# Dhole/collaborative_filtering

Hardware: AMD Instinct MI355X
Metric: user-subgraph eigendecomps/sec + predicted ratings/sec, 1M users avg deg 100 (higher is better)
Workload: dtype f32 (eigen) / f64 (predict)

## Files before the change

### collaborative_filtering_amd/_native.py

```python
from __future__ import annotations

import ctypes
import os
from ctypes import POINTER, c_char_p, c_double, c_float, c_int, c_int32, c_uint32, c_uint64, c_void_p

_HERE = os.path.dirname(os.path.abspath(__file__))
LIB_PATH = os.environ.get("CF_MI355X_LIB") or os.path.join(_HERE, "libcf_mi355x.so")
HOST_LIB_PATH = os.path.join(_HERE, "libcf_host.so")

CF_OK = 0
CF_EINVAL = -1
CF_ERANGE = -4
CF_SVD_MAX_NV = 256
CF_ALS_MAX_D = 64
CF_TOPN_MAX_N = 1024
CF_SIGS_OWN = 0
CF_SIGS_COMPAT = 1
CF_MAX_K = 192
CF_SPILL_MAX_K = 5000
CF_EIGEN_TRIDIAG = 0
CF_EIGEN_JACOBI = 1
CF_GRAPH_DENSE = 0
CF_GRAPH_CSR = 1
CF_FILTER_CHEBY = 0
CF_FILTER_BINOMIAL = 1

SIGNATURES = {
    "cf_version": (c_int, []),
    "cf_device_count": (c_int, []),
    "cf_create": (c_int, [c_int, POINTER(c_void_p)]),
    "cf_destroy": (None, [c_void_p]),
    "cf_release_workspaces": (c_int, [c_void_p]),
    "cf_last_error": (c_char_p, [c_void_p]),
    "cf_set_jacobi": (c_int, [c_void_p, c_float, c_int]),
    "cf_set_eigen_refine": (c_int, [c_void_p, c_int, c_float, c_float]),
    "cf_set_eigen_split": (c_int, [c_void_p, c_int]),
    "cf_set_pred_pack": (c_int, [c_void_p, c_int]),
    "cf_debug_split_schedule": (c_int, [c_int, c_int, POINTER(c_int), POINTER(c_int), POINTER(c_int), POINTER(c_int)]),
    "cf_set_step_masks": (c_int, [c_void_p, c_int]),
    "cf_set_local_wlim": (c_int, [c_void_p, c_int]),
    "cf_debug_predict_nmax": (c_int, [c_int]),
    "cf_set_knn2_topk": (c_int, [c_void_p, c_uint32]),
    "cf_set_eigen_method": (c_int, [c_void_p, c_int]),
    "cf_debug_stats": (c_int, [c_void_p, c_int, c_void_p]),
    "cf_eigen_bucket_timing": (c_int, [c_void_p, c_int, c_void_p]),
    "cf_eigen_bucket_timing_split": (c_int, [c_void_p, c_int, c_void_p, c_void_p]),
    "cf_debug_phases": (c_int, [c_void_p, c_int, c_void_p]),
    "cf_debug_spill": (c_int, [c_void_p, c_int, c_void_p]),
    "cf_debug_tri": (c_int, [c_void_p, c_int, c_void_p]),
    "cf_item_graph_upload": (c_int, [c_void_p, c_uint32, c_void_p, c_void_p, c_void_p]),
    "cf_item_graph_upload_dense": (c_int, [c_void_p, c_uint32, c_void_p, c_int]),
    "cf_item_graph_device": (c_void_p, [c_void_p, POINTER(c_uint32)]),
    "cf_set_graph_layout": (c_int, [c_void_p, c_int]),
    "cf_graph_info": (c_int, [c_void_p, c_void_p, c_void_p, c_void_p]),
    "cf_item_cosine_edges": (c_int, [c_void_p, c_uint32, c_uint32, c_void_p, c_void_p, c_void_p, c_float, c_int, c_int,
                                     c_void_p, c_void_p, c_void_p, c_uint64, c_void_p]),
    "cf_plan_create": (c_int, [c_void_p, c_uint32, c_void_p, POINTER(c_void_p)]),
    "cf_plan_destroy": (None, [c_void_p]),
    "cf_evec_slots": (c_uint64, [c_uint32]),
# ... 189 lines not shown
```

### collaborative_filtering_amd/api.py

```python
from __future__ import annotations

from ctypes import byref, c_double, c_float, c_int, c_uint32, c_void_p
from dataclasses import dataclass

import numpy as np

from . import _native
from ._native import CF_ERANGE, CF_FILTER_BINOMIAL, CF_FILTER_CHEBY, CF_SIGS_COMPAT, CF_SIGS_OWN, NativeError, ptr


def _check(lib, ctx, rc, what):
    if rc != _native.CF_OK:
        msg = lib.cf_last_error(ctx)
        raise NativeError(f"{what} failed ({rc}): {msg.decode() if msg else ''}")


def evec_offsets(item_off: np.ndarray) -> tuple[np.ndarray, int]:
    k = np.diff(item_off.astype(np.int64))
    slots = k * np.maximum(k, 2)
    off = np.zeros(len(k), dtype=np.uint64)
    if len(k):
        off[1:] = np.cumsum(slots)[:-1]
    return off, int(slots.sum())

# ... 211 lines not shown
        self.close()

    def __del__(self):
        try:
            self.close()
        except Exception:
            pass

    def _chk(self, rc, what):
        _check(self.lib, self.h, rc, what)

    def set_eigen_method(self, method: str = "jacobi"):
        code = {"tridiag": _native.CF_EIGEN_TRIDIAG, "jacobi": _native.CF_EIGEN_JACOBI}[method]
        self._chk(self.lib.cf_set_eigen_method(self.h, code), "cf_set_eigen_method")

    def set_jacobi(self, tol_scale: float = 1.0, max_sweeps: int = 30):
        self._chk(self.lib.cf_set_jacobi(self.h, tol_scale, max_sweeps), "cf_set_jacobi")

    def set_eigen_refine(self, enable: bool = True, stop_rel: float = 1e-3, delta: float = 1e-2):
        self._chk(self.lib.cf_set_eigen_refine(self.h, int(enable), stop_rel, delta), "cf_set_eigen_refine")

    def set_eigen_split(self, enable=True):
        self._chk(self.lib.cf_set_eigen_split(self.h, int(enable)), "cf_set_eigen_split")

    def set_pred_pack(self, mode=1):
        self._chk(self.lib.cf_set_pred_pack(self.h, int(mode)), "cf_set_pred_pack")

    def set_local_wlim(self, bisect: bool = True):
        self._chk(self.lib.cf_set_local_wlim(self.h, int(bisect)), "cf_set_local_wlim")

    def set_step_masks(self, enable: bool = True):
        self._chk(self.lib.cf_set_step_masks(self.h, int(enable)), "cf_set_step_masks")

    def debug_stats(self, enable: bool = True, read: bool = False):
        out = np.zeros(8, dtype=np.uint64) if read else None
        self._chk(self.lib.cf_debug_stats(self.h, int(enable), ptr(out)), "cf_debug_stats")
        if read:
            n = max(int(out[1]), 1)
            return {"sweeps_mean": int(out[0]) / n, "users": int(out[1]), "sweeps_max": int(out[2]),
                    "capped": int(out[3]), "assembly_cyc_per_user": int(out[4]) / n,
                    "jacobi_cyc_per_user": int(out[5]) / n, "epilogue_cyc_per_user": int(out[6]) / n,
                    "jacobi_cyc_per_step": int(out[5]) / max(int(out[7]), 1)}
        return None

    def eigen_bucket_timing(self, enable: bool = True, read: bool = False, sweeps: bool = False):
        out = np.zeros(13, dtype=np.float32) if read else None
# ... 795 lines not shown
```

### collaborative_filtering_amd/csrc/cf_eigen.hip

```cpp

#include "cf_eigen_common.h"

namespace {
using namespace cf_eig;

template <int EMAX, bool NARROW = false>
struct EigenGeom {
    static constexpr int NR = 16 * EMAX;
    static constexpr int NC = NARROW ? 188 : NR;
    static constexpr int E2 = NR / (2 * kGroup);
    static constexpr int LD16 = NR + ((16 - NR) % 64 + 64) % 64;
    static constexpr int LD = (NC * LD16 + 9 * NR <= 40960 - 4) ? LD16 : NR + 8;
    static constexpr int NT = (NR > 128) ? 1024 : 512;
    static constexpr int WPE = EMAX <= 5 ? 6 : 4;

    static constexpr size_t bytes() {
        return sizeof(float) * (size_t)NC * LD
               + sizeof(uint32_t) * NR
               + sizeof(float) * NR * 5
               + sizeof(int) * NR
               + sizeof(int) * 4;
    }
};
static_assert(EigenGeom<12, true>::LD % 64 == 16, "narrow bucket-12 layout must be conflict-free");
static_assert(EigenGeom<12, true>::bytes() <= 163840, "narrow bucket-12 layout exceeds 160 KiB LDS");

template <int EMAX, bool NARROW = false, bool RESUME = false>
__global__ __launch_bounds__((EigenGeom<EMAX, NARROW>::NT), (EigenGeom<EMAX, NARROW>::WPE)) void eigen_kernel(EigenArgs a) {
    using G = EigenGeom<EMAX, NARROW>;
    constexpr int NR = G::NR;
    constexpr int LD = G::LD;
    auto bidx = [](int i, int j) { return j * LD + i; };
    constexpr int E2 = G::E2;
    constexpr int NT = G::NT;
    extern __shared__ float smem[];
    float* B = smem;
    uint32_t* s_item = reinterpret_cast<uint32_t*>(B + (size_t)G::NC * LD);
    float* s_s = reinterpret_cast<float*>(s_item + NR);
    float* s_l2d = s_s + NR;
    float* s_sig = s_l2d + NR;
    float* s_mu = s_sig + NR;
    float* s_dev = s_mu + NR;
    int* s_perm = reinterpret_cast<int*>(s_dev + NR);
    int* s_flag = s_perm + NR;

    const int tid = threadIdx.x;
    const int lane = tid & 63;
    const int wave = tid >> 6;
    constexpr int NW = NT / 64;
    unsigned long long t_phase0 = (a.stats && tid == 0) ? __builtin_amdgcn_s_memtime() : 0ull;
    unsigned long long t_phase1 = 0, t_phase2 = 0;
    const int mode = a.mode;
    if (a.only_flag && !a.only_flag[blockIdx.x]) return;
    const uint32_t unit = a.order[a.first + blockIdx.x];
// ... 99 lines not shown
            const float si = s_s[i];
            for (int j = lane; j < k; j += 64)
                L2m[(size_t)i * k + j] = (j == i) ? s_l2d[i] : -(si * B[bidx(i, j)]) * s_s[j];
        }
    }
    __syncthreads();

    for (int j = wave; j < k; j += NW) {
        const float sj = s_s[j];
        for (int i = j + 1 + lane; i < k; i += 64) {
            const float v = -(s_s[i] * B[bidx(i, j)]) * sj;
            B[bidx(i, j)] = v;
            B[bidx(j, i)] = v;
        }
        if (lane == 0) B[bidx(j, j)] = s_l2d[j] + 1.0f;
    }
    for (int i = tid; i < k; i += NT) s_dev[i] = 0.0f;
    if (tid == 0) s_flag[0] = 0;
    __syncthreads();
    }

    if (a.stats && tid == 0) t_phase1 = __builtin_amdgcn_s_memtime();
    const int n = (k + 1) & ~1;
    const int g = tid / kGroup;
    const int lig = tid % kGroup;
    const float tol = a.tol_scale * sqrtf((float)k) * 2.384185791015625e-07f;
    const float tol2 = tol * tol;
    const bool refine = mode == kUser && a.refine && k > 1;
    const float stop2 = refine ? a.stop_rel * a.stop_rel : kSigRot2 * tol2;
    const float close2 = refine ? a.close_sigrot * a.close_sigrot * tol2 : stop2;
    const float dclose2 = refine ? 2.0f * a.refine_delta * a.refine_delta : -1.0f;
    float* s_nrm = s_l2d;
    constexpr int NG = NT / kGroup;
    int sweep = 0;
    if constexpr (!RESUME) {
    for (; sweep < a.max_sweeps && k > 1; ++sweep) {
        for (int c = g; c < k; c += NG) {
            const f2* bc = reinterpret_cast<const f2*>(B + c * LD);
            f2 acc = {0.f, 0.f};
#pragma unroll
            for (int e = 0; e < E2; ++e) {
                const f2 x = lds_ld(bc + kGroup * e + lig);
                acc = __builtin_elementwise_fma(x, x, acc);
            }
            const float nc = pair_sum(acc.x + acc.y);
            if (lig == 0) s_nrm[c] = nc;
        }
        __syncthreads();
        if (a.sort_sweeps) {
            int* s_map = s_perm;
            const bool asc = a.sort_sweeps == 2;
            {
                constexpr int RB = (NR + 63) / 64;
                float ni[RB];
#pragma unroll
                for (int r = 0; r < RB; ++r) ni[r] = (64 * r + lane < k) ? s_nrm[64 * r + lane] : -1.0f;
                for (int j = wave; j < k; j += NW) {
                    const float nj = s_nrm[j];
                    int rank = 0;
#pragma unroll
                    for (int r = 0; r < RB; ++r) {
                        const int i = 64 * r + lane;
                        const bool before = asc ? ni[r] < nj : ni[r] > nj;
                        rank += __popcll(__ballot(i < k && (before || (ni[r] == nj && i < j))));
                    }
                    if (lane == 0) s_map[rank] = j;
                }
            }
// ... 26 lines not shown
                    }
                }
                if (tid < k) {
                    s_dev[tid] = dv;
                    s_nrm[tid] = nv;
                }
                __syncthreads();
            }
        }
        for (int L = 0;; ++L) {
            const int segmax = (n + (1 << L) - 1) >> L;
            if (segmax < 2) break;
            const int FL = (segmax + 1) >> 1;
            const int sigma = g / FL, fi = g - sigma * FL;
            int s0 = 0, s1 = n;
            for (int bit = L - 1; bit >= 0; --bit) {
                const int half = (s1 - s0 + 1) >> 1;
                if ((sigma >> bit) & 1) s0 += half;
                else s1 = s0 + half;
            }
            const int f = (s1 - s0 + 1) >> 1, t = (s1 - s0) - f;
            const int p = s0 + fi;
            const bool fixed = sigma < (1 << L) && fi < f && p < k;
            auto slot = [&](int, int e) { return kGroup * e + lig; };
            f2* bp = reinterpret_cast<f2*>(B + (fixed ? p : 0) * LD);
            f2 xp[E2];
            float devp = 0.0f, al = 0.0f;
            bool pmod = false;
            if (fixed) {
                f2 al2 = {0.f, 0.f};
#pragma unroll
                for (int e = 0; e < E2; ++e) {
                    xp[e] = lds_ld(bp + slot(p, e));
                    al2 = __builtin_elementwise_fma(xp[e], xp[e], al2);
                }
                devp = s_dev[p];
                al = pair_sum(al2.x + al2.y);
            }
            const int tv = fixed ? min(t, k - s0 - f) : 0;
            const int nlive = fixed ? f : 0;
            int ti = fi;
            f2* bq = reinterpret_cast<f2*>(B + (s0 + f + ti) * LD);
            f2* const bq0 = reinterpret_cast<f2*>(B + (s0 + f) * LD);
            for (int step = 0; step < FL; ++step) {
                const int q = s0 + f + ti;
                if (step < nlive && ti < tv) {
                    const float dq = s_dev[q];
                    const float be = s_nrm[q];
                    f2 xq[E2];
                    f2 ga2[2] = {{0.f, 0.f}, {0.f, 0.f}};
#pragma unroll
                    for (int e = 0; e < E2; ++e) xq[e] = lds_ld(bq + slot(q, e));
#pragma unroll
                    for (int e = 0; e < E2; ++e) ga2[e & 1] = __builtin_elementwise_fma(xp[e], xq[e], ga2[e & 1]);
                    const f2 gs = ga2[0] + ga2[1];
                    const float ga = pair_sum(gs.x + gs.y);
                    if (ga * ga > tol2 * (al * be)) {
                        const float dd = be - al;
                        const float r = __builtin_amdgcn_sqrtf(fmaf(dd, dd, 4.0f * ga * ga));
                        const float tt = (dd < 0.0f ? -2.0f * ga : 2.0f * ga) * __builtin_amdgcn_rcpf(fabsf(dd) + r);
                        const float c = __builtin_amdgcn_rsqf(fmaf(tt, tt, 1.0f));
                        const float sn = c * tt;
                        const f2 c2 = {c, c}, s2 = {sn, sn}, ns2 = {-sn, -sn};
#pragma unroll
                        for (int e = 0; e < E2; ++e) {
                            const f2 np = __builtin_elementwise_fma(ns2, xq[e], c2 * xp[e]);
                            lds_st(bq + slot(q, e), __builtin_elementwise_fma(s2, xp[e], c2 * xq[e]));
                            xp[e] = np;
                        }
                        const float delta = fmaf(sn, sn, fmaf(c, c, -1.0f));
                        const float cc = c * c, ss = sn * sn;
                        const float ndp = delta + fmaf(cc, devp, ss * dq);
                        const float csg = 2.0f * c * sn * ga;
                        const float nal = fmaf(cc, al, fmaf(ss, be, -csg));
                        if (lig == 0) {
                            s_dev[q] = delta + fmaf(ss, devp, cc * dq);
                            s_nrm[q] = fmaf(ss, al, fmaf(cc, be, csg));
                            const float g2 = ga * ga, ab = al * be, dab = be - al;
                            if (g2 > stop2 * ab || (g2 > close2 * ab && dab * dab <= dclose2 * (al + be)))
                                s_flag[0] = 1;
                        }
                        devp = ndp;
                        al = nal;
                        pmod = true;
                    }
                }
                __syncthreads();
                bq += LD / 2;
                if (++ti == f) {
                    ti = 0;
                    bq = bq0;
                }
            }
            if (pmod) {
#pragma unroll
                for (int e = 0; e < E2; ++e) lds_st(bp + slot(p, e), xp[e]);
                if (lig == 0) {
                    s_dev[p] = devp;
                    s_nrm[p] = al;
                }
            }
            __syncthreads();
        }
        const int rotated = s_flag[0];
        __syncthreads();
        if (!rotated) break;
        if (tid == 0) s_flag[0] = 0;
        __syncthreads();
    }
    }
    if (a.stats && tid == 0) t_phase2 = __builtin_amdgcn_s_memtime();
    if (!RESUME && a.stats && tid == 0) {
        atomicAdd(&a.stats[0], (unsigned long long)(sweep + 1));
        atomicAdd(&a.stats[1], 1ull);
        atomicMax(&a.stats[2], (unsigned long long)(sweep + 1));
        if (sweep >= a.max_sweeps) atomicAdd(&a.stats[3], 1ull);
    }

    if (refine) {
        for (int c = g; c < k; c += NG) {
            const f2* bc = reinterpret_cast<const f2*>(B + c * LD);
            f2 acc = {0.f, 0.f};
#pragma unroll
            for (int e = 0; e < E2; ++e) {
                const f2 x = lds_ld(bc + kGroup * e + lig);
                acc = __builtin_elementwise_fma(x, x, acc);
            }
            const float nc = pair_sum(acc.x + acc.y);
            if (lig == 0) s_mu[c] = nc / (1.0f + s_dev[c]);
        }
        __syncthreads();
        const int nb = (k + 15) >> 4;
        const int m16 = lane & 15, kq = lane >> 4;
        const int j = wave * 16 + m16;
        const bool jv = wave < nb && j < k;
        constexpr int HB = (EMAX + 1) / 2;
        f4 kv[EMAX];
#pragma unroll
        for (int I = 0; I < EMAX; ++I) kv[I] = f4{0.f, 0.f, 0.f, 0.f};
        if (wave < nb) {
            const f4* pj = reinterpret_cast<const f4*>(B + (jv ? j : 0) * LD + 4 * kq);
            for (int c = 0; c < nb; ++c) {
                const f4 y = jv ? pj[4 * c] : f4{0.f, 0.f, 0.f, 0.f};
#pragma unroll
                for (int I0 = 0; I0 < EMAX; I0 += 4) {
                    f4 x[4];
#pragma unroll
                    for (int g4 = 0; g4 < 4; ++g4) {
                        const int ci = (I0 + g4) * 16 + m16;
                        x[g4] = (I0 + g4 < nb && ci < k) ? reinterpret_cast<const f4*>(B + ci * LD + 4 * kq)[4 * c]
                                                         : f4{0.f, 0.f, 0.f, 0.f};
                    }
#pragma unroll
                    for (int t = 0; t < 4; ++t)
#pragma unroll
                        for (int g4 = 0; g4 < 4; ++g4)
                            if (I0 + g4 < EMAX && I0 + g4 < nb)
                                kv[I0 + g4] = __builtin_amdgcn_mfma_f32_16x16x4f32(x[g4][t], y[t], kv[I0 + g4], 0, 0, 0);
                }
            }
            const float muj2 = jv ? s_mu[j] : 1.0f;
            const float muj = sqrtf(muj2);
            const float dlt = a.refine_delta;
            float ksq = 0.0f;
#pragma unroll
            for (int I = 0; I < EMAX; ++I)
#pragma unroll
                for (int r = 0; r < 4; ++r) {
                    const int i = I * 16 + 4 * kq + r;
                    float kvv = 0.0f;
                    if (I < nb && jv && i < k && i != j) {
                        const float mui2 = s_mu[i];
                        if (fabsf(sqrtf(mui2) - muj) > dlt) kvv = kv[I][r] / (mui2 - muj2);
                    }
                    kv[I][r] = -kvv;
                    ksq = fmaf(kvv, kvv, ksq);
                }
            ksq += __shfl_xor(ksq, 16);
            ksq += __shfl_xor(ksq, 32);
            if (kq == 0 && jv) s_dev[j] += ksq;
        }
#pragma unroll
        for (int h = 0; h < 2; ++h) {
            f4 out[HB];
            if (wave < nb) {
#pragma unroll
                for (int q = 0; q < HB; ++q) {
                    const int R = h * HB + q;
                    out[q] = (jv && R < nb) ? *reinterpret_cast<const f4*>(B + j * LD + R * 16 + 4 * kq)
                                            : f4{0.f, 0.f, 0.f, 0.f};
                }
#pragma unroll
                for (int I = 0; I < EMAX; ++I) {
                    if (I < nb) {
#pragma unroll
                        for (int t = 0; t < 4; ++t) {
                            const int c = I * 16 + 4 * kq + t;
                            const float* bc = B + c * LD + h * HB * 16 + m16;
#pragma unroll
                            for (int q = 0; q < HB; ++q) {
                                if (h * HB + q < nb) {
                                    const float av = c < k ? bc[q * 16] : 0.0f;
                                    out[q] = __builtin_amdgcn_mfma_f32_16x16x4f32(av, kv[I][t], out[q], 0, 0, 0);
                                }
                            }
                        }
                    }
                }
            }
            __syncthreads();
            if (jv) {
#pragma unroll
                for (int q = 0; q < HB; ++q) {
                    const int R = h * HB + q;
                    if (R < nb) *reinterpret_cast<f4*>(B + j * LD + R * 16 + 4 * kq) = out[q];
                }
            }
        }
        __syncthreads();
    }

    for (int j = g; j < k; j += NG) {
        const f2* bc = reinterpret_cast<const f2*>(B + j * LD);
        double acc = 0.0, sum = 0.0;
#pragma unroll
        for (int e = 0; e < E2; ++e) {
            const f2 x = lds_ld(bc + kGroup * e + lig);
            acc = fma((double)x.x, (double)x.x, acc);
            acc = fma((double)x.y, (double)x.y, acc);
            sum += (double)x.x;
            sum += (double)x.y;
        }
#pragma unroll
        for (int o = 1; o < kGroup; o <<= 1) {
            acc += __shfl_xor(acc, o);
            sum += __shfl_xor(sum, o);
        }
        if (lig == 0) {
            const double nrm = sqrt(acc);
            s_mu[j] = (float)(nrm / sqrt(1.0 + (double)s_dev[j]));
            s_s[j] = (float)((sum < 0.0 ? -1.0 : 1.0) / nrm);
        }
    }
    __syncthreads();
    if (mode == kSigma) {
        if (tid == 0) {
            float smin = s_mu[0];
            for (int j = 1; j < k; ++j) smin = fminf(smin, s_mu[j]);
            a.wlim[unit] = smin;
        }
        return;
    }
    for (int j = tid; j < k; j += NT) {
        const float mj = s_mu[j];
        int rank = 0;
        for (int i = 0; i < k; ++i) {
            const float mi = s_mu[i];
// ... 35 lines not shown
    for (int idx = tid; idx < k * m; idx += NT) {
        const int i = idx / m;
        const int r = idx - i * m;
        float v = 0.0f;
        if (r < k) {
            const int j = s_perm[r];
            v = B[bidx(i, j)] * s_s[j];
        }
        out[idx] = v;
    }
    if (a.stats && tid == 0) {
        const unsigned long long t3 = __builtin_amdgcn_s_memtime();
        atomicAdd(&a.stats[6], t3 - t_phase2);
        if constexpr (!RESUME) {
            atomicAdd(&a.stats[4], t_phase1 - t_phase0);
            atomicAdd(&a.stats[5], t_phase2 - t_phase1);
            int steps = 0;
            for (int L = 0; ((n + (1 << L) - 1) >> L) >= 2; ++L) steps += (((n + (1 << L) - 1) >> L) + 1) >> 1;
            atomicAdd(&a.stats[7], (unsigned long long)((sweep + 1) * steps));
        }
    }
}

template <int EMAX, bool NARROW = false, bool RESUME = false>
int launch_bucket_k(cf_ctx* ctx, const EigenArgs& args, uint32_t count, hipStream_t stream) {
    using G = EigenGeom<EMAX, NARROW>;
    const size_t lds = G::bytes();
    static_assert(G::bytes() <= 163840, "eigen bucket exceeds 160 KiB LDS");
    static bool configured = false;
    if (!configured) {
        CF_HIP_CHECK(ctx, hipFuncSetAttribute((const void*)eigen_kernel<EMAX, NARROW, RESUME>,
                                              hipFuncAttributeMaxDynamicSharedMemorySize, (int)lds));
        configured = true;
    }
    hipLaunchKernelGGL((eigen_kernel<EMAX, NARROW, RESUME>), dim3(count), dim3(G::NT), lds, stream, args);
    CF_HIP_CHECK(ctx, hipGetLastError());
    return CF_OK;
}

template <int EMAX, bool NARROW = false>
int launch_bucket(cf_ctx* ctx, const EigenArgs& args, uint32_t count, hipStream_t stream, uint32_t kmax = 0) {
    if constexpr (EMAX >= kSplitEmaxLow) {
        bool handled = false, finished = false;
        CF_TRY(launch_split_sweeps(ctx, args, EMAX, count, kmax, stream, &handled, &finished));
        if (handled && finished) return CF_OK;
        if (handled) {
            if (ctx->split_mid_ev) {
                CF_HIP_CHECK(ctx, hipEventRecord(ctx->split_mid_ev, stream));
                ctx->split_mid_recorded = true;
            }
            return launch_bucket_k<EMAX, NARROW, true>(ctx, args, count, stream);
        }
    }
    return launch_bucket_k<EMAX, NARROW, false>(ctx, args, count, stream);
}

int launch_bucket12_layout(cf_ctx* ctx, const EigenArgs& args, uint32_t count, uint32_t kmax, hipStream_t stream) {
    static const bool narrow_on = [] {
        const char* e = getenv("CF_EIGEN_NARROW");
        return !(e && e[0] == '0');
// ... 112 lines not shown
        if (timed) {
            CF_HIP_CHECK(ctx, hipEventRecord(ctx->bucket_ev[slot][b.emax][1], stream));
            ctx->bucket_recorded[slot][b.emax] = true;
            ctx->bucket_mid[slot][b.emax] = ctx->split_mid_recorded;
            ctx->split_mid_ev = nullptr;
        }
    }
    if (ctx->bucket_timing && args.mode == kUser) ++ctx->bucket_run;
    return CF_OK;
}

int launch_all_buckets(cf_ctx* ctx, const cf_plan* plan, EigenArgs args, hipStream_t caller) {
    const bool overlap = args.mode == kUser && !args.stats;
    if (overlap) CF_TRY(eigen_fork(ctx, caller));
    const int rc = launch_buckets_on(ctx, plan, args, caller, overlap);
    if (overlap) {
        int rj = eigen_join(ctx, caller);
        const int rs = cf_spill_join(ctx, caller);
        if (rj == CF_OK) rj = rs;
        if (rc == CF_OK) return rj;
    }
    return rc;
}
}

extern "C" int cf_eigen_bucket_timing_split(cf_ctx* ctx, int enable, float* ms13, float* sweeps_ms13) {
    if (!ctx) return CF_EINVAL;
    CF_TRY(set_device(ctx));
    ctx->split_mid_ev = nullptr;
    if (enable && !ctx->bucket_ev[0][1][0])
        for (auto& run : ctx->bucket_ev)
            for (auto& pr : run)
                for (hipEvent_t& e : pr) CF_HIP_CHECK(ctx, hipEventCreate(&e));
    if (ms13) {
        for (int e = 0; e < 13; ++e) {
            double sum = 0.0, sum_a = 0.0;
            int cnt = 0, cnt_a = 0;
            for (int r = 0; r < cf_ctx::kBucketRuns; ++r) {
                if (!ctx->bucket_recorded[r][e]) continue;
                float ms = 0.0f;
                CF_HIP_CHECK(ctx, hipEventSynchronize(ctx->bucket_ev[r][e][1]));
                CF_HIP_CHECK(ctx, hipEventElapsedTime(&ms, ctx->bucket_ev[r][e][0], ctx->bucket_ev[r][e][1]));
                sum += ms;
                ++cnt;
                if (ctx->bucket_mid[r][e]) {
                    CF_HIP_CHECK(ctx, hipEventElapsedTime(&ms, ctx->bucket_ev[r][e][0], ctx->bucket_ev[r][e][2]));
// ... 179 lines not shown
```

### collaborative_filtering_amd/csrc/cf_eigen_common.h

```cpp
#pragma once

#include "cf_internal.h"

namespace cf_eig {

constexpr int kGroup = 8;
#ifndef CF_EIGEN_SIGROT2
#define CF_EIGEN_SIGROT2 256.0f
#endif
constexpr float kSigRot2 = CF_EIGEN_SIGROT2;

using f2 = __attribute__((ext_vector_type(2))) float;
using f4 = __attribute__((ext_vector_type(4))) float;
__device__ __forceinline__ f2 lds_ld(const f2* p) {
    return *(const volatile __attribute__((address_space(3))) f2*)(p);
}
__device__ __forceinline__ void lds_st(f2* p, f2 v) {
#if defined(CF_EIGEN_FUSED_ST) && CF_EIGEN_FUSED_ST
    *p = v;
#else
    *(volatile __attribute__((address_space(3))) f2*)(p) = v;
#endif
}


template <int CTRL>
__device__ __forceinline__ float dpp_mov(float x) {
    return __int_as_float(__builtin_amdgcn_update_dpp(0, __float_as_int(x), CTRL, 0xF, 0xF, false));
}

__device__ __forceinline__ float pair_sum(float x) {
    x += dpp_mov<0xB1>(x);
    x += dpp_mov<0x4E>(x);
    x += dpp_mov<0x141>(x);
    return x;
}

enum EigenMode : int { kUser = 0, kLocal = 1, kSigma = 2 };

struct EigenArgs {
    int mode;
    const uint32_t* order;
    uint32_t first;
    const uint64_t* item_off;
    const uint32_t* items;
    GraphDev graph;
    uint64_t n_items;
    const uint64_t* evec_off;
    int32_t* m_out;
    float* sigs;
    float* evals;
    float* evecs;
    float tol_scale;
    int max_sweeps;
    int refine;
    float stop_rel;
    float refine_delta;
    float close_sigrot;
// ... 40 lines not shown
```

### collaborative_filtering_amd/csrc/cf_internal.h

```cpp
#pragma once

#include <hip/hip_runtime.h>

#include <algorithm>
#include <cstdint>
#include <string>
#include <vector>

#include "cf_abi.h"

struct GraphRow {
    const float* dense;
    const uint32_t* col;
    const float* w;
    uint32_t len;
    __device__ __forceinline__ float operator[](uint32_t b) const {
        if (dense) return dense[b];
        uint32_t lo = 0, hi = len;
        while (lo < hi) {
            const uint32_t mid = (lo + hi) >> 1;
            if (col[mid] < b) lo = mid + 1;
            else hi = mid;
        }
        return (lo < len && col[lo] == b) ? w[lo] : 0.0f;
// ... 78 lines not shown
    size_t knn_part_bytes = 0;
    uint32_t knn_chunk_users = 0;
    uint32_t knn2_topk = 0;
    int knn_chunks = 0;
    void* d_prep = nullptr;
    size_t prep_bytes = 0;
    hipEvent_t prep_ev[2] = {nullptr, nullptr};
    static constexpr int kAuxStreams = 2;
    hipStream_t aux_stream[kAuxStreams] = {};
    hipEvent_t aux_event[kAuxStreams + 1] = {};
    static constexpr int kBucketRuns = 16;
    bool bucket_timing = false;
    hipEvent_t bucket_ev[kBucketRuns][13][3] = {};
    bool bucket_recorded[kBucketRuns][13] = {};
    bool bucket_mid[kBucketRuns][13] = {};
    hipEvent_t split_mid_ev = nullptr;
    bool split_mid_recorded = false;
    int bucket_run = 0;
    hipStream_t step_stream[2] = {};
    hipEvent_t step_bucket_ev[16] = {};
    hipEvent_t step_sync_ev[4] = {};
    hipEvent_t step_time_ev[3] = {};
    uint32_t* d_split_sched[13] = {};
    int eigen_split = -1;
    int pred_pack = -1;
    int split_finish = -1;
    float filter_ms = 0.0f;
    uint64_t filter_nnz = 0;
    void* d_als = nullptr;
    size_t als_bytes = 0;
    float sgd_reduce_ms[2] = {0.0f, 0.0f};
    float svdpp_reduce_ms[3] = {0.0f, 0.0f, 0.0f};
    uint32_t topn_block = 0;
};

constexpr int kSpillBucket = -1;

struct cf_bucket {
    int emax = 0;

    uint32_t count = 0;
    uint32_t first = 0;
    uint32_t kmax = 0;
};

struct cf_tri_chunk {
// ... 191 lines not shown
```

### include/cf_abi.h

```cpp
#ifndef CF_ABI_H
#define CF_ABI_H

#include <stddef.h>
#include <stdint.h>

#ifdef __cplusplus
extern "C" {
#endif

#define CF_OK 0
#define CF_EINVAL (-1)
#define CF_ENOMEM (-2)
#define CF_EHIP (-3)
#define CF_ERANGE (-4)
#define CF_ESTATE (-5)

#define CF_MAX_K 192
#define CF_SPILL_MAX_K 5000

typedef struct cf_ctx cf_ctx;
typedef struct cf_plan cf_plan;

int cf_version(void);
int cf_device_count(void);
int cf_create(int device, cf_ctx** out);
void cf_destroy(cf_ctx* ctx);
int cf_release_workspaces(cf_ctx* ctx);
const char* cf_last_error(const cf_ctx* ctx);
#define CF_EIGEN_TRIDIAG 0
#define CF_EIGEN_JACOBI 1
int cf_set_eigen_method(cf_ctx* ctx, int method);
int cf_set_jacobi(cf_ctx* ctx, float tol_scale, int max_sweeps);
int cf_set_eigen_refine(cf_ctx* ctx, int enable, float stop_rel, float delta);
int cf_set_eigen_split(cf_ctx* ctx, int enable);
int cf_set_pred_pack(cf_ctx* ctx, int mode);
int cf_debug_split_schedule(int emax, int k, int* steps, int* levels, int* max_groups, int* max_slots);
int cf_set_step_masks(cf_ctx* ctx, int enable);
int cf_set_local_wlim(cf_ctx* ctx, int bisect);
int cf_debug_stats(cf_ctx* ctx, int enable, uint64_t* out8);
int cf_debug_spill(cf_ctx* ctx, int enable, uint64_t* out8);
int cf_debug_tri(cf_ctx* ctx, int enable, uint64_t* out8);
int cf_debug_phases(cf_ctx* ctx, int enable, uint64_t* out16);
int cf_debug_predict_nmax(int lmax);
int cf_eigen_bucket_timing(cf_ctx* ctx, int enable, float* ms13);
int cf_eigen_bucket_timing_split(cf_ctx* ctx, int enable, float* ms13, float* sweeps_ms13);

#define CF_GRAPH_DENSE 0
#define CF_GRAPH_CSR 1
int cf_set_graph_layout(cf_ctx* ctx, int layout);
int cf_graph_info(const cf_ctx* ctx, int* layout, uint32_t* n_items, uint64_t* nnz);
int cf_item_graph_upload(cf_ctx* ctx, uint32_t n_items, const uint64_t* row_ptr,
                         const uint32_t* col, const float* w);
int cf_item_graph_upload_dense(cf_ctx* ctx, uint32_t n_items, const float* w_dense,
                               int on_device);
const float* cf_item_graph_device(const cf_ctx* ctx, uint32_t* n_items);

int cf_plan_create(cf_ctx* ctx, uint32_t n_users, const uint64_t* item_off, cf_plan** out);
// ... 270 lines not shown
```

Measured before the change: 336,400.

## Use four lanes per column pair in one-sided Jacobi for mid-size eigen buckets

```diff
diff --git a/collaborative_filtering_amd/_native.py b/collaborative_filtering_amd/_native.py
--- a/collaborative_filtering_amd/_native.py
+++ b/collaborative_filtering_amd/_native.py
@@ -35,6 +35,9 @@
     "cf_set_jacobi": (c_int, [c_void_p, c_float, c_int]),
     "cf_set_eigen_refine": (c_int, [c_void_p, c_int, c_float, c_float]),
     "cf_set_eigen_split": (c_int, [c_void_p, c_int]),
+    "cf_set_eigen_lanes": (c_int, [c_void_p, c_int]),
+    "cf_debug_eigen_geometry": (c_int, [c_int, c_int, POINTER(c_int), POINTER(c_int), POINTER(c_int), POINTER(c_int),
+                                        POINTER(c_int)]),
     "cf_set_pred_pack": (c_int, [c_void_p, c_int]),
     "cf_debug_split_schedule": (c_int, [c_int, c_int, POINTER(c_int), POINTER(c_int), POINTER(c_int), POINTER(c_int)]),
     "cf_set_step_masks": (c_int, [c_void_p, c_int]),
diff --git a/collaborative_filtering_amd/api.py b/collaborative_filtering_amd/api.py
--- a/collaborative_filtering_amd/api.py
+++ b/collaborative_filtering_amd/api.py
@@ -257,6 +257,9 @@
 
     def set_eigen_split(self, enable=True):
         self._chk(self.lib.cf_set_eigen_split(self.h, int(enable)), "cf_set_eigen_split")
+
+    def set_eigen_lanes(self, lanes=0):
+        self._chk(self.lib.cf_set_eigen_lanes(self.h, int(lanes)), "cf_set_eigen_lanes")
 
     def set_pred_pack(self, mode=1):
         self._chk(self.lib.cf_set_pred_pack(self.h, int(mode)), "cf_set_pred_pack")
diff --git a/collaborative_filtering_amd/csrc/cf_eigen.hip b/collaborative_filtering_amd/csrc/cf_eigen.hip
--- a/collaborative_filtering_amd/csrc/cf_eigen.hip
+++ b/collaborative_filtering_amd/csrc/cf_eigen.hip
@@ -4,15 +4,23 @@
 namespace {
 using namespace cf_eig;
 
-template <int EMAX, bool NARROW = false>
+template <int EMAX, bool NARROW = false, int LANES = kGroup>
 struct EigenGeom {
+    static_assert(LANES == 8 || (LANES == 4 && EMAX <= 8 && !NARROW), "4 lanes per pair: buckets 1-8 only");
     static constexpr int NR = 16 * EMAX;
     static constexpr int NC = NARROW ? 188 : NR;
+    static constexpr int SUB = kGroup / LANES;
     static constexpr int E2 = NR / (2 * kGroup);
     static constexpr int LD16 = NR + ((16 - NR) % 64 + 64) % 64;
-    static constexpr int LD = (NC * LD16 + 9 * NR <= 40960 - 4) ? LD16 : NR + 8;
-    static constexpr int NT = (NR > 128) ? 1024 : 512;
-    static constexpr int WPE = EMAX <= 5 ? 6 : 4;
+    static constexpr int LD48 = NR + ((48 - NR) % 64 + 64) % 64;
+    static constexpr int LD = EMAX <= 8 ? (LD48 < LD16 ? LD48 : LD16)
+                                        : ((NC * LD16 + 9 * NR <= 40960 - 4) ? LD16 : NR + 8);
+    static constexpr int NG = EMAX > 8 ? 128 : EMAX > 4 ? 64 : EMAX > 2 ? 32 : 16;
+    static constexpr int NT = NG * LANES;
+    static constexpr int NW = NT / 64;
+    static constexpr int WPE = EMAX > 8 ? 4
+                               : LANES == 8 ? (EMAX <= 5 ? 6 : 4)
+                               : (EMAX <= 4 ? 6 : EMAX == 5 ? 5 : EMAX <= 7 ? 3 : 2);
 
     static constexpr size_t bytes() {
         return sizeof(float) * (size_t)NC * LD
@@ -21,15 +29,21 @@
                + sizeof(int) * NR
                + sizeof(int) * 4;
     }
+    static constexpr int UPC_LDS = (int)(163840 / bytes());
+    static constexpr int UPC = UPC_LDS < 4 * WPE / NW ? UPC_LDS : 4 * WPE / NW;
 };
+static_assert(EigenGeom<9>::NT == 1024 && EigenGeom<12, true>::NT == 1024 && EigenGeom<8>::NT == 512, "block sizes");
+static_assert(EigenGeom<7, false, 4>::bytes() * 3 <= 163840 && EigenGeom<4, false, 4>::bytes() * 7 <= 163840 &&
+                  EigenGeom<5, false, 4>::bytes() * 5 <= 163840, "users per CU the LDS holds");
 static_assert(EigenGeom<12, true>::LD % 64 == 16, "narrow bucket-12 layout must be conflict-free");
 static_assert(EigenGeom<12, true>::bytes() <= 163840, "narrow bucket-12 layout exceeds 160 KiB LDS");
 
-template <int EMAX, bool NARROW = false, bool RESUME = false>
-__global__ __launch_bounds__((EigenGeom<EMAX, NARROW>::NT), (EigenGeom<EMAX, NARROW>::WPE)) void eigen_kernel(EigenArgs a) {
-    using G = EigenGeom<EMAX, NARROW>;
+template <int EMAX, bool NARROW = false, bool RESUME = false, int LANES = kGroup>
+__global__ __launch_bounds__((EigenGeom<EMAX, NARROW, LANES>::NT), (EigenGeom<EMAX, NARROW, LANES>::WPE)) void eigen_kernel(EigenArgs a) {
+    using G = EigenGeom<EMAX, NARROW, LANES>;
     constexpr int NR = G::NR;
     constexpr int LD = G::LD;
+    constexpr int SUB = G::SUB;
     auto bidx = [](int i, int j) { return j * LD + i; };
     constexpr int E2 = G::E2;
     constexpr int NT = G::NT;
@@ -175,8 +189,8 @@
 
     if (a.stats && tid == 0) t_phase1 = __builtin_amdgcn_s_memtime();
     const int n = (k + 1) & ~1;
-    const int g = tid / kGroup;
-    const int lig = tid % kGroup;
+    const int g = tid / LANES;
+    const int lig = tid % LANES;
     const float tol = a.tol_scale * sqrtf((float)k) * 2.384185791015625e-07f;
     const float tol2 = tol * tol;
     const bool refine = mode == kUser && a.refine && k > 1;
@@ -184,19 +198,28 @@
     const float close2 = refine ? a.close_sigrot * a.close_sigrot * tol2 : stop2;
     const float dclose2 = refine ? 2.0f * a.refine_delta * a.refine_delta : -1.0f;
     float* s_nrm = s_l2d;
-    constexpr int NG = NT / kGroup;
+    auto col_norm2 = [&](const f2* bc) {
+        f2 acc[SUB];
+#pragma unroll
+        for (int s = 0; s < SUB; ++s) acc[s] = f2{0.f, 0.f};
+#pragma unroll
+        for (int e = 0; e < E2; ++e) {
+            f2 x[SUB];
+            col_ld<SUB>(bc, e, x);
+#pragma unroll
+            for (int s = 0; s < SUB; ++s) acc[s] = __builtin_elementwise_fma(x[s], x[s], acc[s]);
+        }
+        float part[SUB];
+#pragma unroll
+        for (int s = 0; s < SUB; ++s) part[s] = acc[s].x + acc[s].y;
+        return group_sum<SUB>(part);
+    };
+    constexpr int NG = G::NG;
     int sweep = 0;
     if constexpr (!RESUME) {
     for (; sweep < a.max_sweeps && k > 1; ++sweep) {
         for (int c = g; c < k; c += NG) {
-            const f2* bc = reinterpret_cast<const f2*>(B + c * LD);
-            f2 acc = {0.f, 0.f};
-#pragma unroll
-            for (int e = 0; e < E2; ++e) {
-                const f2 x = lds_ld(bc + kGroup * e + lig);
-                acc = __builtin_elementwise_fma(x, x, acc);
-            }
-            const float nc = pair_sum(acc.x + acc.y);
+            const float nc = col_norm2(reinterpret_cast<const f2*>(B + c * LD) + SUB * lig);
             if (lig == 0) s_nrm[c] = nc;
         }
         __syncthreads();
@@ -269,39 +292,54 @@
             const int f = (s1 - s0 + 1) >> 1, t = (s1 - s0) - f;
             const int p = s0 + fi;
             const bool fixed = sigma < (1 << L) && fi < f && p < k;
-            auto slot = [&](int, int e) { return kGroup * e + lig; };
-            f2* bp = reinterpret_cast<f2*>(B + (fixed ? p : 0) * LD);
-            f2 xp[E2];
+            f2* bp = reinterpret_cast<f2*>(B + (fixed ? p : 0) * LD) + SUB * lig;
+            f2 xp[E2][SUB];
             float devp = 0.0f, al = 0.0f;
             bool pmod = false;
             if (fixed) {
-                f2 al2 = {0.f, 0.f};
+                f2 al2[SUB];
+#pragma unroll
+                for (int s = 0; s < SUB; ++s) al2[s] = f2{0.f, 0.f};
 #pragma unroll
                 for (int e = 0; e < E2; ++e) {
-                    xp[e] = lds_ld(bp + slot(p, e));
-                    al2 = __builtin_elementwise_fma(xp[e], xp[e], al2);
+                    col_ld<SUB>(bp, e, xp[e]);
+#pragma unroll
+                    for (int s = 0; s < SUB; ++s) al2[s] = __builtin_elementwise_fma(xp[e][s], xp[e][s], al2[s]);
                 }
                 devp = s_dev[p];
-                al = pair_sum(al2.x + al2.y);
+                float part[SUB];
+#pragma unroll
+                for (int s = 0; s < SUB; ++s) part[s] = al2[s].x + al2[s].y;
+                al = group_sum<SUB>(part);
             }
             const int tv = fixed ? min(t, k - s0 - f) : 0;
             const int nlive = fixed ? f : 0;
             int ti = fi;
-            f2* bq = reinterpret_cast<f2*>(B + (s0 + f + ti) * LD);
-            f2* const bq0 = reinterpret_cast<f2*>(B + (s0 + f) * LD);
+            f2* bq = reinterpret_cast<f2*>(B + (s0 + f + ti) * LD) + SUB * lig;
+            f2* const bq0 = reinterpret_cast<f2*>(B + (s0 + f) * LD) + SUB * lig;
             for (int step = 0; step < FL; ++step) {
                 const int q = s0 + f + ti;
                 if (step < nlive && ti < tv) {
                     const float dq = s_dev[q];
                     const float be = s_nrm[q];
-                    f2 xq[E2];
-                    f2 ga2[2] = {{0.f, 0.f}, {0.f, 0.f}};
-#pragma unroll
-                    for (int e = 0; e < E2; ++e) xq[e] = lds_ld(bq + slot(q, e));
-#pragma unroll
-                    for (int e = 0; e < E2; ++e) ga2[e & 1] = __builtin_elementwise_fma(xp[e], xq[e], ga2[e & 1]);
-                    const f2 gs = ga2[0] + ga2[1];
-                    const float ga = pair_sum(gs.x + gs.y);
+                    f2 xq[E2][SUB];
+                    f2 ga2[SUB][2];
+#pragma unroll
+                    for (int s = 0; s < SUB; ++s) ga2[s][0] = ga2[s][1] = f2{0.f, 0.f};
+#pragma unroll
+                    for (int e = 0; e < E2; ++e) col_ld<SUB>(bq, e, xq[e]);
+#pragma unroll
+                    for (int e = 0; e < E2; ++e)
+#pragma unroll
+                        for (int s = 0; s < SUB; ++s)
+                            ga2[s][e & 1] = __builtin_elementwise_fma(xp[e][s], xq[e][s], ga2[s][e & 1]);
+                    float gpart[SUB];
+#pragma unroll
+                    for (int s = 0; s < SUB; ++s) {
+                        const f2 gs = ga2[s][0] + ga2[s][1];
+                        gpart[s] = gs.x + gs.y;
+                    }
+                    const float ga = group_sum<SUB>(gpart);
                     if (ga * ga > tol2 * (al * be)) {
                         const float dd = be - al;
                         const float r = __builtin_amdgcn_sqrtf(fmaf(dd, dd, 4.0f * ga * ga));
@@ -311,9 +349,14 @@
                         const f2 c2 = {c, c}, s2 = {sn, sn}, ns2 = {-sn, -sn};
 #pragma unroll
                         for (int e = 0; e < E2; ++e) {
-                            const f2 np = __builtin_elementwise_fma(ns2, xq[e], c2 * xp[e]);
-                            lds_st(bq + slot(q, e), __builtin_elementwise_fma(s2, xp[e], c2 * xq[e]));
-                            xp[e] = np;
+                            f2 nq[SUB];
+#pragma unroll
+                            for (int s = 0; s < SUB; ++s) {
+                                const f2 np = __builtin_elementwise_fma(ns2, xq[e][s], c2 * xp[e][s]);
+                                nq[s] = __builtin_elementwise_fma(s2, xp[e][s], c2 * xq[e][s]);
+                                xp[e][s] = np;
+                            }
+                            col_st<SUB>(bq, e, nq);
                         }
                         const float delta = fmaf(sn, sn, fmaf(c, c, -1.0f));
                         const float cc = c * c, ss = sn * sn;
@@ -341,7 +384,7 @@
             }
             if (pmod) {
 #pragma unroll
-                for (int e = 0; e < E2; ++e) lds_st(bp + slot(p, e), xp[e]);
+                for (int e = 0; e < E2; ++e) col_st<SUB>(bp, e, xp[e]);
                 if (lig == 0) {
                     s_dev[p] = devp;
                     s_nrm[p] = al;
@@ -366,89 +409,94 @@
 
     if (refine) {
         for (int c = g; c < k; c += NG) {
-            const f2* bc = reinterpret_cast<const f2*>(B + c * LD);
-            f2 acc = {0.f, 0.f};
-#pragma unroll
-            for (int e = 0; e < E2; ++e) {
-                const f2 x = lds_ld(bc + kGroup * e + lig);
-                acc = __builtin_elementwise_fma(x, x, acc);
-            }
-            const float nc = pair_sum(acc.x + acc.y);
+            const float nc = col_norm2(reinterpret_cast<const f2*>(B + c * LD) + SUB * lig);
             if (lig == 0) s_mu[c] = nc / (1.0f + s_dev[c]);
         }
         __syncthreads();
         const int nb = (k + 15) >> 4;
         const int m16 = lane & 15, kq = lane >> 4;
-        const int j = wave * 16 + m16;
-        const bool jv = wave < nb && j < k;
+        constexpr int TPW = (EMAX + NW - 1) / NW;
         constexpr int HB = (EMAX + 1) / 2;
-        f4 kv[EMAX];
-#pragma unroll
-        for (int I = 0; I < EMAX; ++I) kv[I] = f4{0.f, 0.f, 0.f, 0.f};
-        if (wave < nb) {
-            const f4* pj = reinterpret_cast<const f4*>(B + (jv ? j : 0) * LD + 4 * kq);
-            for (int c = 0; c < nb; ++c) {
-                const f4 y = jv ? pj[4 * c] : f4{0.f, 0.f, 0.f, 0.f};
-#pragma unroll
-                for (int I0 = 0; I0 < EMAX; I0 += 4) {
-                    f4 x[4];
-#pragma unroll
-                    for (int g4 = 0; g4 < 4; ++g4) {
-                        const int ci = (I0 + g4) * 16 + m16;
-                        x[g4] = (I0 + g4 < nb && ci < k) ? reinterpret_cast<const f4*>(B + ci * LD + 4 * kq)[4 * c]
-                                                         : f4{0.f, 0.f, 0.f, 0.f};
+        f4 kv[TPW][EMAX];
+#pragma unroll
+        for (int tt = 0; tt < TPW; ++tt) {
+            const int J = wave + tt * NW;
+            const int j = J * 16 + m16;
+            const bool jv = J < nb && j < k;
+#pragma unroll
+            for (int I = 0; I < EMAX; ++I) kv[tt][I] = f4{0.f, 0.f, 0.f, 0.f};
+            if (J < nb) {
+                const f4* pj = reinterpret_cast<const f4*>(B + (jv ? j : 0) * LD + 4 * kq);
+                for (int c = 0; c < nb; ++c) {
+                    const f4 y = jv ? pj[4 * c] : f4{0.f, 0.f, 0.f, 0.f};
+#pragma unroll
+                    for (int I0 = 0; I0 < EMAX; I0 += 4) {
+                        f4 x[4];
+#pragma unroll
+                        for (int g4 = 0; g4 < 4; ++g4) {
+                            const int ci = (I0 + g4) * 16 + m16;
+                            x[g4] = (I0 + g4 < nb && ci < k) ? reinterpret_cast<const f4*>(B + ci * LD + 4 * kq)[4 * c]
+                                                             : f4{0.f, 0.f, 0.f, 0.f};
+                        }
+#pragma unroll
+                        for (int t = 0; t < 4; ++t)
+#pragma unroll
+                            for (int g4 = 0; g4 < 4; ++g4)
+                                if (I0 + g4 < EMAX && I0 + g4 < nb)
+                                    kv[tt][I0 + g4] =
+                                        __builtin_amdgcn_mfma_f32_16x16x4f32(x[g4][t], y[t], kv[tt][I0 + g4], 0, 0, 0);
                     }
-#pragma unroll
-                    for (int t = 0; t < 4; ++t)
-#pragma unroll
-                        for (int g4 = 0; g4 < 4; ++g4)
-                            if (I0 + g4 < EMAX && I0 + g4 < nb)
-                                kv[I0 + g4] = __builtin_amdgcn_mfma_f32_16x16x4f32(x[g4][t], y[t], kv[I0 + g4], 0, 0, 0);
                 }
-            }
-            const float muj2 = jv ? s_mu[j] : 1.0f;
-            const float muj = sqrtf(muj2);
-            const float dlt = a.refine_delta;
-            float ksq = 0.0f;
-#pragma unroll
-            for (int I = 0; I < EMAX; ++I)
-#pragma unroll
-                for (int r = 0; r < 4; ++r) {
-                    const int i = I * 16 + 4 * kq + r;
-                    float kvv = 0.0f;
-                    if (I < nb && jv && i < k && i != j) {
-                        const float mui2 = s_mu[i];
-                        if (fabsf(sqrtf(mui2) - muj) > dlt) kvv = kv[I][r] / (mui2 - muj2);
+                const float muj2 = jv ? s_mu[j] : 1.0f;
+                const float muj = sqrtf(muj2);
+                const float dlt = a.refine_delta;
+                float ksq = 0.0f;
+#pragma unroll
+                for (int I = 0; I < EMAX; ++I)
+#pragma unroll
+                    for (int r = 0; r < 4; ++r) {
+                        const int i = I * 16 + 4 * kq + r;
+                        float kvv = 0.0f;
+                        if (I < nb && jv && i < k && i != j) {
+                            const float mui2 = s_mu[i];
+                            if (fabsf(sqrtf(mui2) - muj) > dlt) kvv = kv[tt][I][r] / (mui2 - muj2);
+                        }
+                        kv[tt][I][r] = -kvv;
+                        ksq = fmaf(kvv, kvv, ksq);
                     }
-                    kv[I][r] = -kvv;
-                    ksq = fmaf(kvv, kvv, ksq);
-                }
-            ksq += __shfl_xor(ksq, 16);
-            ksq += __shfl_xor(ksq, 32);
-            if (kq == 0 && jv) s_dev[j] += ksq;
+                ksq += __shfl_xor(ksq, 16);
+                ksq += __shfl_xor(ksq, 32);
+                if (kq == 0 && jv) s_dev[j] += ksq;
+            }
         }
 #pragma unroll
         for (int h = 0; h < 2; ++h) {
-            f4 out[HB];
-            if (wave < nb) {
-#pragma unroll
-                for (int q = 0; q < HB; ++q) {
-                    const int R = h * HB + q;
-                    out[q] = (jv && R < nb) ? *reinterpret_cast<const f4*>(B + j * LD + R * 16 + 4 * kq)
-                                            : f4{0.f, 0.f, 0.f, 0.f};
-                }
-#pragma unroll
-                for (int I = 0; I < EMAX; ++I) {
-                    if (I < nb) {
-#pragma unroll
-                        for (int t = 0; t < 4; ++t) {
-                            const int c = I * 16 + 4 * kq + t;
-                            const float* bc = B + c * LD + h * HB * 16 + m16;
-#pragma unroll
-                            for (int q = 0; q < HB; ++q) {
-                                if (h * HB + q < nb) {
-                                    const float av = c < k ? bc[q * 16] : 0.0f;
-                                    out[q] = __builtin_amdgcn_mfma_f32_16x16x4f32(av, kv[I][t], out[q], 0, 0, 0);
+            f4 out[TPW][HB];
+#pragma unroll
+            for (int tt = 0; tt < TPW; ++tt) {
+                const int J = wave + tt * NW;
+                const int j = J * 16 + m16;
+                const bool jv = J < nb && j < k;
+                if (J < nb) {
+#pragma unroll
+                    for (int q = 0; q < HB; ++q) {
+                        const int R = h * HB + q;
+                        out[tt][q] = (jv && R < nb) ? *reinterpret_cast<const f4*>(B + j * LD + R * 16 + 4 * kq)
+                                                    : f4{0.f, 0.f, 0.f, 0.f};
+                    }
+#pragma unroll
+                    for (int I = 0; I < EMAX; ++I) {
+                        if (I < nb) {
+#pragma unroll
+                            for (int t = 0; t < 4; ++t) {
+                                const int c = I * 16 + 4 * kq + t;
+                                const float* bc = B + c * LD + h * HB * 16 + m16;
+#pragma unroll
+                                for (int q = 0; q < HB; ++q) {
+                                    if (h * HB + q < nb) {
+                                        const float av = c < k ? bc[q * 16] : 0.0f;
+                                        out[tt][q] = __builtin_amdgcn_mfma_f32_16x16x4f32(av, kv[tt][I][t], out[tt][q], 0, 0, 0);
+                                    }
                                 }
                             }
                         }
@@ -456,11 +504,16 @@
                 }
             }
             __syncthreads();
-            if (jv) {
-#pragma unroll
-                for (int q = 0; q < HB; ++q) {
-                    const int R = h * HB + q;
-                    if (R < nb) *reinterpret_cast<f4*>(B + j * LD + R * 16 + 4 * kq) = out[q];
+#pragma unroll
+            for (int tt = 0; tt < TPW; ++tt) {
+                const int J = wave + tt * NW;
+                const int j = J * 16 + m16;
+                if (J < nb && j < k) {
+#pragma unroll
+                    for (int q = 0; q < HB; ++q) {
+                        const int R = h * HB + q;
+                        if (R < nb) *reinterpret_cast<f4*>(B + j * LD + R * 16 + 4 * kq) = out[tt][q];
+                    }
                 }
             }
         }
@@ -468,18 +521,29 @@
     }
 
     for (int j = g; j < k; j += NG) {
-        const f2* bc = reinterpret_cast<const f2*>(B + j * LD);
-        double acc = 0.0, sum = 0.0;
+        const f2* bc = reinterpret_cast<const f2*>(B + j * LD) + SUB * lig;
+        double accs[SUB], sums[SUB];
+#pragma unroll
+        for (int s = 0; s < SUB; ++s) accs[s] = sums[s] = 0.0;
 #pragma unroll
         for (int e = 0; e < E2; ++e) {
-            const f2 x = lds_ld(bc + kGroup * e + lig);
-            acc = fma((double)x.x, (double)x.x, acc);
-            acc = fma((double)x.y, (double)x.y, acc);
-            sum += (double)x.x;
-            sum += (double)x.y;
-        }
-#pragma unroll
-        for (int o = 1; o < kGroup; o <<= 1) {
+            f2 x[SUB];
+            col_ld<SUB>(bc, e, x);
+#pragma unroll
+            for (int s = 0; s < SUB; ++s) {
+                accs[s] = fma((double)x[s].x, (double)x[s].x, accs[s]);
+                accs[s] = fma((double)x[s].y, (double)x[s].y, accs[s]);
+                sums[s] += (double)x[s].x;
+                sums[s] += (double)x[s].y;
+            }
+        }
+        double acc = accs[0], sum = sums[0];
+        if constexpr (SUB == 2) {
+            acc += accs[1];
+            sum += sums[1];
+        }
+#pragma unroll
+        for (int o = 1; o < LANES; o <<= 1) {
             acc += __shfl_xor(acc, o);
             sum += __shfl_xor(sum, o);
         }
@@ -561,20 +625,47 @@
     }
 }
 
+constexpr int kDefaultLanes[13] = {0, 8, 8, 8, 8, 4, 4, 4, 8, 8, 8, 8, 8};
+
+constexpr int lanes_of(int emax, int setting) {
+    if (emax > 8) return 8;
+    return setting == 0 ? kDefaultLanes[emax] : setting;
+}
+
+int eigen_lanes_setting(cf_ctx* ctx) {
+    if (ctx->eigen_lanes < 0) {
+        const char* e = getenv("CF_EIGEN_LANES");
+        const int v = e ? atoi(e) : 0;
+        ctx->eigen_lanes = (v == 4 || v == 8) ? v : 0;
+    }
+    return ctx->eigen_lanes;
+}
+
+template <int EMAX, bool NARROW, bool RESUME, int LANES>
+int launch_bucket_kl(cf_ctx* ctx, const EigenArgs& args, uint32_t count, hipStream_t stream) {
+    using G = EigenGeom<EMAX, NARROW, LANES>;
+    const size_t lds = G::bytes();
+    static_assert(G::bytes() <= 163840, "eigen bucket exceeds 160 KiB LDS");
+    static_assert(G::bytes() * G::UPC <= 163840, "intended users per CU exceed the LDS");
+    static_assert(G::NT >= G::NR && G::NT <= 1024, "block size");
+    static bool configured = false;
+    if (!configured) {
+        CF_HIP_CHECK(ctx, hipFuncSetAttribute((const void*)eigen_kernel<EMAX, NARROW, RESUME, LANES>,
+                                              hipFuncAttributeMaxDynamicSharedMemorySize, (int)lds));
+        configured = true;
+    }
+    hipLaunchKernelGGL((eigen_kernel<EMAX, NARROW, RESUME, LANES>), dim3(count), dim3(G::NT), lds, stream, args);
+    CF_HIP_CHECK(ctx, hipGetLastError());
+    return CF_OK;
+}
+
 template <int EMAX, bool NARROW = false, bool RESUME = false>
 int launch_bucket_k(cf_ctx* ctx, const EigenArgs& args, uint32_t count, hipStream_t stream) {
-    using G = EigenGeom<EMAX, NARROW>;
-    const size_t lds = G::bytes();
-    static_assert(G::bytes() <= 163840, "eigen bucket exceeds 160 KiB LDS");
-    static bool configured = false;
-    if (!configured) {
-        CF_HIP_CHECK(ctx, hipFuncSetAttribute((const void*)eigen_kernel<EMAX, NARROW, RESUME>,
-                                              hipFuncAttributeMaxDynamicSharedMemorySize, (int)lds));
-        configured = true;
-    }
-    hipLaunchKernelGGL((eigen_kernel<EMAX, NARROW, RESUME>), dim3(count), dim3(G::NT), lds, stream, args);
-    CF_HIP_CHECK(ctx, hipGetLastError());
-    return CF_OK;
+    if constexpr (EMAX <= 8 && !NARROW && !RESUME) {
+        if (lanes_of(EMAX, eigen_lanes_setting(ctx)) == 4)
+            return launch_bucket_kl<EMAX, NARROW, RESUME, 4>(ctx, args, count, stream);
+    }
+    return launch_bucket_kl<EMAX, NARROW, RESUME, 8>(ctx, args, count, stream);
 }
 
 template <int EMAX, bool NARROW = false>
@@ -733,6 +824,58 @@
     }
     return rc;
 }
+}
+
+extern "C" int cf_set_eigen_lanes(cf_ctx* ctx, int lanes) {
+    if (!ctx) return CF_EINVAL;
+    if (lanes != 0 && lanes != 4 && lanes != 8) return CF_EINVAL;
+    ctx->eigen_lanes = lanes;
+    return CF_OK;
+}
+
+namespace {
+template <int EMAX, int LANES>
+void geometry_of(int* threads, int* ld, int* lds_bytes, int* users_per_cu) {
+    using G = EigenGeom<EMAX, false, LANES>;
+    *threads = G::NT;
+    *ld = G::LD;
+    *lds_bytes = (int)G::bytes();
+    *users_per_cu = G::UPC;
+}
+template <int EMAX>
+void geometry_of_lanes(int lanes, int* threads, int* ld, int* lds_bytes, int* users_per_cu) {
+    if constexpr (EMAX <= 8) {
+        if (lanes == 4) return geometry_of<EMAX, 4>(threads, ld, lds_bytes, users_per_cu);
+    }
+    geometry_of<EMAX, 8>(threads, ld, lds_bytes, users_per_cu);
+}
+}
+
+extern "C" int cf_debug_eigen_geometry(int emax, int lanes_setting, int* lanes, int* threads, int* ld,
+                                       int* lds_bytes, int* users_per_cu) {
+    if (emax < 1 || emax > 12 || (lanes_setting != 0 && lanes_setting != 4 && lanes_setting != 8)) return CF_EINVAL;
+    const int l = lanes_of(emax, lanes_setting);
+    int t = 0, d = 0, b = 0, u = 0;
+    switch (emax) {
+        case 1: geometry_of_lanes<1>(l, &t, &d, &b, &u); break;
+        case 2: geometry_of_lanes<2>(l, &t, &d, &b, &u); break;
+        case 3: geometry_of_lanes<3>(l, &t, &d, &b, &u); break;
+        case 4: geometry_of_lanes<4>(l, &t, &d, &b, &u); break;
+        case 5: geometry_of_lanes<5>(l, &t, &d, &b, &u); break;
+        case 6: geometry_of_lanes<6>(l, &t, &d, &b, &u); break;
+        case 7: geometry_of_lanes<7>(l, &t, &d, &b, &u); break;
+        case 8: geometry_of_lanes<8>(l, &t, &d, &b, &u); break;
+        case 9: geometry_of_lanes<9>(l, &t, &d, &b, &u); break;
+        case 10: geometry_of_lanes<10>(l, &t, &d, &b, &u); break;
+        case 11: geometry_of_lanes<11>(l, &t, &d, &b, &u); break;
+        default: geometry_of_lanes<12>(l, &t, &d, &b, &u); break;
+    }
+    if (lanes) *lanes = l;
+    if (threads) *threads = t;
+    if (ld) *ld = d;
+    if (lds_bytes) *lds_bytes = b;
+    if (users_per_cu) *users_per_cu = u;
+    return CF_OK;
 }
 
 extern "C" int cf_eigen_bucket_timing_split(cf_ctx* ctx, int enable, float* ms13, float* sweeps_ms13) {
diff --git a/collaborative_filtering_amd/csrc/cf_eigen_common.h b/collaborative_filtering_amd/csrc/cf_eigen_common.h
--- a/collaborative_filtering_amd/csrc/cf_eigen_common.h
+++ b/collaborative_filtering_amd/csrc/cf_eigen_common.h
@@ -34,6 +34,43 @@
     x += dpp_mov<0x4E>(x);
     x += dpp_mov<0x141>(x);
     return x;
+}
+
+__device__ __forceinline__ f4 lds_ld4(const f4* p) {
+    return *(const volatile __attribute__((address_space(3))) f4*)(p);
+}
+__device__ __forceinline__ void lds_st4(f4* p, f4 v) {
+    *(volatile __attribute__((address_space(3))) f4*)(p) = v;
+}
+
+template <int SUB>
+__device__ __forceinline__ void col_ld(const f2* col, int e, f2 (&x)[SUB]) {
+    if constexpr (SUB == 1) {
+        x[0] = lds_ld(col + kGroup * e);
+    } else {
+        const f4 v = lds_ld4(reinterpret_cast<const f4*>(col + kGroup * e));
+        x[0] = f2{v.x, v.y};
+        x[1] = f2{v.z, v.w};
+    }
+}
+template <int SUB>
+__device__ __forceinline__ void col_st(f2* col, int e, const f2 (&x)[SUB]) {
+    if constexpr (SUB == 1) {
+        lds_st(col + kGroup * e, x[0]);
+    } else {
+        lds_st4(reinterpret_cast<f4*>(col + kGroup * e), f4{x[0].x, x[0].y, x[1].x, x[1].y});
+    }
+}
+template <int SUB>
+__device__ __forceinline__ float group_sum(const float (&s)[SUB]) {
+    if constexpr (SUB == 1) {
+        return pair_sum(s[0]);
+    } else {
+        float x = s[0] + s[1];
+        x += dpp_mov<0xB1>(x);
+        x += dpp_mov<0x4E>(x);
+        return x;
+    }
 }
 
 enum EigenMode : int { kUser = 0, kLocal = 1, kSigma = 2 };
diff --git a/collaborative_filtering_amd/csrc/cf_internal.h b/collaborative_filtering_amd/csrc/cf_internal.h
--- a/collaborative_filtering_amd/csrc/cf_internal.h
+++ b/collaborative_filtering_amd/csrc/cf_internal.h
@@ -124,6 +124,7 @@
     hipEvent_t step_sync_ev[4] = {};
     hipEvent_t step_time_ev[3] = {};
     uint32_t* d_split_sched[13] = {};
+    int eigen_lanes = -1;
     int eigen_split = -1;
     int pred_pack = -1;
     int split_finish = -1;
diff --git a/include/cf_abi.h b/include/cf_abi.h
--- a/include/cf_abi.h
+++ b/include/cf_abi.h
@@ -33,6 +33,9 @@
 int cf_set_jacobi(cf_ctx* ctx, float tol_scale, int max_sweeps);
 int cf_set_eigen_refine(cf_ctx* ctx, int enable, float stop_rel, float delta);
 int cf_set_eigen_split(cf_ctx* ctx, int enable);
+int cf_set_eigen_lanes(cf_ctx* ctx, int lanes);
+int cf_debug_eigen_geometry(int emax, int lanes_setting, int* lanes, int* threads, int* ld, int* lds_bytes,
+                            int* users_per_cu);
 int cf_set_pred_pack(cf_ctx* ctx, int mode);
 int cf_debug_split_schedule(int emax, int k, int* steps, int* levels, int* max_groups, int* max_slots);
 int cf_set_step_masks(cf_ctx* ctx, int enable);
```

Measured after the change: 348,700, median of 6. 3.7% higher.
